# pytorch/ELF

Hardware: AMD Instinct MI355X
Metric: mcts_rollouts_per_sec (self-play, 19x19 Go, 8192 rollouts/move, bs 16) (higher is better)
Workload: dtype f32; 1 GPU; BASELINE configs[2]: MCTS self-play bs=16, 8192 rollouts/move, 20x256 fp16 net on PyTorch-ROCm, 2048 games/GPU in 1 group(s), window crosses a move boundary; games_per_gpu=2048, groups=1, board_size=19, mcts_threads=1, net_dtype=fp16, moves_in_window=2048, nodes_per_game=12288, node_bytes=6626, live_nodes=6241478, largest_tree=8184

## Files before the change

elf_amd/_lib.py:

```python
import ctypes as C
import os

HERE = os.path.dirname(os.path.abspath(__file__))
LIB_PATH = os.path.join(HERE, "lib", "libelf_amd.so")
ZOBRIST_BIN = os.path.join(HERE, "data", "zobrist21.bin")

_lib = None

KERNEL_SOURCES = ("go_board.cuh", "mcts.cuh", "train.cuh", "stl_emul.h", "engine_host.h", "elf_amd.hip", "mcts_capi.hip", "train_capi.hip",
                  "net_epilogue.hip", "Makefile")


def kernel_source_hash():
    import hashlib
    h = hashlib.sha256()
    for name in KERNEL_SOURCES:
        with open(os.path.join(HERE, "csrc", name), "rb") as f:
            h.update(name.encode() + b"\0" + f.read() + b"\0")
    return h.hexdigest()[:16]

_vp, _i, _i64, _f, _sz = C.c_void_p, C.c_int, C.c_int64, C.c_float, C.c_size_t
SIGNATURES = {
    "elfgo_create": (_i, [_i, _i, _i, _vp, C.POINTER(_vp)]),
    "elfgo_destroy": (_i, [_vp]),
    "elfgo_board_size": (_i, [_vp]),
    "elfgo_capacity": (_i, [_vp]),
    "elfgo_slot_bytes": (_sz, [_vp]),
    "elfgo_sync": (_i, [_vp, _vp]),
    "elfgo_reset": (_i, [_vp, _vp, _i, _vp]),
    "elfgo_copy": (_i, [_vp, _vp, _vp, _i, _vp]),
    "elfgo_forward": (_i, [_vp, _vp, _vp, _i, _vp, _vp]),
    "elfgo_legal_mask": (_i, [_vp, _vp, _i, _vp, _vp]),
    "elfgo_extract_agz": (_i, [_vp, _vp, _vp, _i, _vp, _i64, _vp]),
    "elfgo_extract_agz_fmt": (_i, [_vp, _vp, _vp, _i, _vp, _i64, _i, _vp]),
    "elfgo_evaluate": (_i, [_vp, _vp, _i, _f, _vp, _vp]),
    "elfgo_info": (_i, [_vp, _vp, _i, _vp, _vp]),
    "elfgo_export_board": (_i, [_vp, _vp, _i, _vp, _vp, _vp]),
    "elfgo_playout": (_i, [_vp, _vp, _vp, _i, _i, _vp, _vp]),
    "elfgo_setup": (_i, [_vp, _vp, _vp, _vp, _i, _vp, _vp]),
    "elfgo_area_map": (_i, [_vp, _vp, _i, _vp, _vp]),
    "elfgo_ladder_map": (_i, [_vp, _vp, _i, _vp, _vp, _vp]),
    "elfgo_own_create": (_i, [_vp, _i, C.POINTER(_vp)]),
    "elfgo_own_destroy": (_i, [_vp]),
    "elfgo_own_scratch_bytes": (_sz, [_vp]),
    "elfgo_own_run": (_i, [_vp, _vp, _vp, _i, _i, _i, _f, _vp, _vp, _vp]),
    "elfmcts_create": (_i, [_vp, _i, _i, _i, _vp, C.POINTER(_vp)]),
    "elfmcts_destroy": (_i, [_vp]),
    "elfmcts_set_options": (_i, [_vp, _vp]),
    "elfmcts_set_feature_format": (_i, [_vp, _i]),
    "elfmcts_get_feature_format": (_i, [_vp, C.POINTER(_i)]),
    "elfmcts_max_rollouts_per_step": (_i, []),
    "elfmcts_set_game_mask": (_i, [_vp, _vp]),
    "elfmcts_set_required_versions": (_i, [_vp, _vp]),
    "elfmcts_num_games": (_i, [_vp]),
    "elfmcts_edge_stride": (_i, [_vp]),
    "elfmcts_node_bytes": (_sz, [_vp]),
    "elfmcts_tree_bytes_per_game": (_sz, [_i, _i]),
    "elfmcts_tree_bytes_per_game2": (_sz, [_i, _i, _i, _i, _i]),
    "elfmcts_pool_info": (_i, [_vp, _vp, _i]),
    "elfmcts_count_live": (_i, [_vp, _vp]),
    "elfmcts_num_threads": (_i, [_vp]),
    "elfmcts_thread_draws": (_i, [_vp, _vp, _vp]),
    "elfmcts_clear": (_i, [_vp, _vp, _i, _vp]),
    "elfmcts_set_root": (_i, [_vp, _vp, _vp]),
    "elfmcts_set_d4": (_i, [_vp, _vp, _vp]),
    "elfmcts_dirichlet": (_i, [_vp, _vp, _vp, _f, _vp]),
    "elfmcts_select": (_i, [_vp, _vp, _vp, _i64, _vp, _vp]),
    "elfmcts_expand": (_i, [_vp, _vp, _i64, _vp, _vp, _i, _vp]),
    "elfmcts_root": (_i, [_vp, _vp, _vp, _vp, _vp, _vp, _vp, _vp]),
    "elfmcts_advance": (_i, [_vp, _vp, _vp]),
    "elfmcts_validate": (_i, [_vp, _vp]),
    "elfmcts_node_visits": (_i, [_vp, _vp]),
    "elfsp_create": (_i, [_vp, _i, _vp, C.POINTER(_vp)]),
    "elfsp_destroy": (_i, [_vp]),
    "elfsp_engine": (_vp, [_vp]),
    "elfsp_mcts": (_vp, [_vp]),
    "elfsp_ts_requests_deferred": (_i64, [_vp]),
    "elfsp_ts_games_deferred": (_i, [_vp]),
    "elfsp_max_rows": (_i, [_vp]),
    "elfsp_max_rows_actor": (_i, [_vp, _i]),
    "elfsp_mcts_actor": (_vp, [_vp, _i]),
    "elfsp_begin_step2": (_i, [_vp, _vp, _i64, _vp, _vp]),
    "elfsp_end_step2": (_i, [_vp, _vp, _i64, _vp, _vp, _vp]),
    "elfsp_last_rows2": (_i, [_vp, _vp]),
    "elfsp_set_request2": (_i, [_vp, _vp]),
    "elfsp_set_request3": (_i, [_vp, _vp, _vp]),
    "elfrec_sgf_parse": (_i, [_i, C.c_char_p, _vp, _vp, _i, _vp]),
    "elfrec_sgf_setup": (_i, [_i, C.c_char_p, _vp, _vp]),
    "elfrec_game_sgf": (_i64, [_vp, _vp, _i, _vp, _i, _f, C.c_char_p, C.c_char_p, C.c_char_p, C.c_char_p, _sz]),
    "elfrec_record_to_sgf": (_i64, [_vp, C.c_char_p, C.c_char_p, C.c_char_p, _sz, C.c_char_p, _sz]),
    "elfrec_client_create": (_i, [C.c_char_p, C.POINTER(_vp)]),
    "elfrec_client_destroy": (_i, [_vp]),
    "elfrec_client_feed": (_i, [_vp, C.c_char_p]),
    "elfrec_client_update_state": (_i, [_vp, _vp]),
    "elfrec_client_size": (_i, [_vp]),
    "elfrec_client_dump_and_clear": (_i64, [_vp, C.c_char_p, _sz]),
    "elfrec_parse_request_seq": (_i, [C.c_char_p, _vp, C.POINTER(_i64), _vp]),
    "elfrec_request_seq_to_json": (_i64, [_vp, _vp, _i64, C.c_char_p, _sz]),
    "elfsp_thread_states": (_i, [_vp, _vp, _i]),
    "elfrq_create": (_i, [_i, _i, _i, C.c_uint32, C.POINTER(_vp)]),
    "elfrq_destroy": (_i, [_vp]),
    "elfrq_insert": (_i, [_vp, C.c_int32, C.c_int32, _i, C.POINTER(C.c_int32)]),
    "elfrq_sizes": (_i, [_vp, _vp]),
    "elfrq_set_threads": (_i, [_vp, _i, _i64, C.c_uint64]),
    "elfrq_draw": (_i, [_vp, _i, _i, _vp, _vp, _vp]),
    "elfsp_progress": (_i, [_vp, _vp]),
    "elfsp_set_pick_seed": (_i, [_vp, C.c_uint32]),
    "elfsp_game_actor": (_i, [_vp, _i]),
    "elfsp_begin_step": (_i, [_vp, _vp, _i64, C.POINTER(_i), _vp]),
    "elfsp_end_step": (_i, [_vp, _vp, _i64, _vp, _vp, _vp]),
    "elfsp_last_rows": (_i, [_vp, C.POINTER(_i)]),
    "elfsp_set_request": (_i, [_vp, _i64, _i64, _f, _f, _i]),
    "elfsp_take_game_starts": (_i, [_vp, C.POINTER(_i64), C.POINTER(_i64)]),
    "elfsp_stats": (_i, [_vp, _vp]),
    "elfsp_games_finished": (_i64, [_vp]),
    "elfsp_search_log": (_i, [_vp, _i, _i, _vp, _vp, _vp, _vp, _vp]),
    "elfsp_play": (_i, [_vp, _vp, _vp]),
    "elfsp_preload": (_i, [_vp, _vp, _i, _i, _vp]),
    "elfsp_restart": (_i, [_vp, _vp, _i, _vp]),
    "elfsp_setup": (_i, [_vp, _vp, _i, _vp, _vp, _vp]),
    "elfsp_undo": (_i, [_vp, _vp, _i, _i, _vp]),
    "elfsp_finish": (_i, [_vp, _vp, _i, _i, _vp]),
    "elfsp_take_finished": (_i, [_vp, _vp, _i]),
    "elfsp_last_score": (_i, [_vp, _vp]),
    "elfsp_last_moves": (_i, [_vp, _vp]),
    "elfsp_records_pending": (_i, [_vp]),
    "elfsp_pop_record": (_i, [_vp, _vp, _sz, C.POINTER(_sz)]),
    "elftrain_create": (_i, [_vp, _i, _i, _i, C.c_uint32, C.POINTER(_vp)]),
    "elftrain_destroy": (_i, [_vp]),
    "elftrain_capacity": (_i, [_vp]),
    "elftrain_max_moves": (_i, [_vp]),
    "elftrain_num_records": (_i, [_vp]),
    "elftrain_put": (_i, [_vp, _i, _vp, _i, _f, _i64, _vp, _i, _vp, _i]),
    "elftrain_put_async": (_i, [_vp, _i, _vp, _i, _f, _i64, _vp, _i, _vp, _i, _vp]),
    "elftrain_set_keep_states": (_i, [_vp, _i]),
    "elftrain_draw": (_i, [_vp, _i, _i, _vp, _vp, _vp, _vp]),
    "elftrain_extract": (_i, [_vp, _vp, _vp, _vp, _i, _vp, _vp]),
    "elfrec_coords_to_sgfstr": (_i, [_i, _vp, _i, _vp, _sz]),
    "elfrec_sgfstr_to_coords": (_i, [_i, C.c_char_p, _vp, _i]),
    "elfrec_record_to_json": (_i, [_vp, _vp, _i, _vp, _i, _vp, _i, _f, _i, _i, C.c_uint64, C.c_uint64, _vp, _sz]),
    "elfrec_record_to_json2": (_i, [_vp, _vp, _vp, _i, _vp, _i, _vp, _i, _f, _i, _i, C.c_uint64, C.c_uint64, _vp, _sz]),
    "elfrec_quantise_policy": (_i, [_i, _vp, _vp, _i, _vp]),
    "elfnet_bias_act_f16": (_i, [_vp, _vp, _vp, _i64, _i, _i, _vp]),
    "elfnet_bias_act_bf16": (_i, [_vp, _vp, _vp, _i64, _i, _i, _vp]),
    "elfnet_conv3x3_f16": (_i, [_vp, _vp, _vp, _vp, _vp, _i64, _i, _i, _i, _i, _i, _i, _vp]),
    "elfgo_set_device": (_i, [_i]),
    "elfgo_get_device": (_i, [C.POINTER(_i)]),
    "elfgo_mem_info": (_i, [_i, C.POINTER(_sz), C.POINTER(_sz)]),
    "elfgo_pointer_kind": (_i, [_vp, C.POINTER(_i)]),
    "elfgo_memcpy2d_async": (_i, [_vp, _sz, _vp, _sz, _sz, _sz, _vp]),
    "elfgo_stream_sync": (_i, [_vp]),
    "elfgo_malloc": (_i, [C.POINTER(_vp), _sz]),
    "elfgo_free": (_i, [_vp]),
    "elfgo_memcpy_h2d": (_i, [_vp, _vp, _sz]),
    "elfgo_memcpy_d2h": (_i, [_vp, _vp, _sz]),
    "elfgo_error_string": (C.c_char_p, [_i]),
    "elfgo_version": (C.c_char_p, []),
}


def lib():
    global _lib
    if _lib is None:
        if not os.path.exists(LIB_PATH):
            raise ImportError(
                "elf_amd: %s not built. Run `python -c 'import __graft_entry__ as g; g.build()'` "
                "(or make -C elf_amd/csrc). There is no CPU fallback." % LIB_PATH
            )
        L = C.CDLL(LIB_PATH)
        for name, (res, args) in SIGNATURES.items():
            f = getattr(L, name)
            f.restype = res
            f.argtypes = args
        _lib = L
    return _lib


class ElfGoError(RuntimeError):
    pass


def check(status):
    if status != 0:
        raise ElfGoError("libelf_amd status %d: %s" % (status, lib().elfgo_error_string(status).decode()))
```

elf_amd/csrc/net_conv.hip:

```cpp
#include <hip/hip_runtime.h>
#include <stdint.h>

#include <array>

#if !__has_include("ck/ck.hpp")
#error "net_conv.hip needs Composable Kernel's headers (ck/ck.hpp, shipped with ROCm under <rocm>/include/ck): there is no build of libelf_amd.so without the fused trunk convolution"
#endif
#include "ck/ck.hpp"
#include "ck/tensor_operation/gpu/device/convolution_forward_specialization.hpp"
#include "ck/tensor_operation/gpu/device/gemm_specialization.hpp"
#include "ck/tensor_operation/gpu/device/impl/device_grouped_conv_fwd_multiple_abd_xdl_cshuffle.hpp"
#include "ck/tensor_operation/gpu/device/tensor_layout.hpp"
#include "ck/tensor_operation/gpu/element/element_wise_operation.hpp"

#include "../../include/elf_amd.h"

namespace {

using F16 = ck::half_t;
using F32 = float;
template <ck::index_t... Is>
using S = ck::Sequence<Is...>;
using PassThrough = ck::tensor_operation::element_wise::PassThrough;
namespace lay = ck::tensor_layout::convolution;

struct BiasResAct {
  int relu;
  template <typename E, typename C, typename D0>
  __host__ __device__ void operator()(E& e, const C& c, const D0& bias) const {
    float v = ck::type_convert<float>(ck::type_convert<F16>(c));
    v += ck::type_convert<float>(bias);
    if (relu) v = fmaxf(v, 0.0f);
    e = ck::type_convert<E>(v);
  }
  template <typename E, typename C, typename D0, typename D1>
  __host__ __device__ void operator()(E& e, const C& c, const D0& bias, const D1& res) const {
    float v = ck::type_convert<float>(ck::type_convert<F16>(c));
    v += ck::type_convert<float>(bias);
    v += ck::type_convert<float>(res);
    if (relu) v = fmaxf(v, 0.0f);
    e = ck::type_convert<E>(v);
  }
};

constexpr auto kConvDefault = ck::tensor_operation::device::ConvolutionForwardSpecialization::Default;
constexpr auto kMNKPadding = ck::tensor_operation::device::GemmSpecialization::MNKPadding;

template <typename DsLayout, typename DsTypes>
using ConvA = ck::tensor_operation::device::DeviceGroupedConvFwdMultipleABD_Xdl_CShuffle<
    2, lay::NHWGC, lay::GKYXC, DsLayout, lay::NHWGK, F16, F16, F32, F16, DsTypes, F16, PassThrough, PassThrough, BiasResAct,
    kConvDefault, kMNKPadding, 1, 256, 256, 128, 32, 8, 8, 32, 32, 4, 2,
    S<4, 64, 1>, S<1, 0, 2>, S<1, 0, 2>, 2, 8, 8, 1,
    S<4, 64, 1>, S<1, 0, 2>, S<1, 0, 2>, 2, 8, 8, 1,
    1, 1, S<1, 32, 1, 8>, 8>;

using DsBias = ck::Tuple<lay::G_K>;
using DsBiasRes = ck::Tuple<lay::G_K, lay::NHWGK>;
using T1 = ck::Tuple<F16>;
using T2 = ck::Tuple<F16, F16>;

struct DevGuard {
  int prev = -1;
  explicit DevGuard(int dev) {
    int cur = -1;
    if (hipGetDevice(&cur) == hipSuccess && cur != dev && hipSetDevice(dev) == hipSuccess) prev = cur;
  }
  ~DevGuard() { if (prev >= 0) (void)hipSetDevice(prev); }
  DevGuard(const DevGuard&) = delete;
  DevGuard& operator=(const DevGuard&) = delete;
};

struct Shape { int n, h, w, c, k; };

template <typename Op, int ND>
int run(const void* x, const void* w, const std::array<const void*, ND>& ds, void* y, const Shape& s, int relu, hipStream_t stream,
        bool launch) {
  using A5 = std::array<ck::index_t, 5>;
  using A2 = std::array<ck::index_t, 2>;
  const int n = s.n, h = s.h, wd = s.w, c = s.c, k = s.k;
  const A5 xl{1, n, c, h, wd}, xs{c, h * wd * c, 1, wd * c, c};
  const A5 wl{1, k, c, 3, 3}, ws{k * 9 * c, 9 * c, 1, 3 * c, c};
  const A5 yl{1, n, k, h, wd}, ys{k, h * wd * k, 1, wd * k, k};
  const A5 bs{k, 0, 1, 0, 0};
  std::array<A5, ND> dl, dst;
  dl[0] = yl; dst[0] = bs;
  if (ND == 2) { dl[ND - 1] = yl; dst[ND - 1] = ys; }
  const A2 one{1, 1};
  try {
    auto arg = Op::MakeArgument(x, w, ds, y, xl, xs, wl, ws, dl, dst, yl, ys, one, one, one, one, PassThrough{}, PassThrough{},
                                BiasResAct{relu});
    if (!Op::IsSupportedArgument(arg)) return ELFGO_E_BADARG;
    if (!launch) return 0;
    auto inv = Op::MakeInvoker();
    (void)inv.Run(arg, StreamConfig{stream, false});
  } catch (...) {
    hipError_t e = hipGetLastError();
    return e == hipSuccess ? (int)hipErrorLaunchFailure : (int)e;
  }
  hipError_t e = hipGetLastError();
  return e == hipSuccess ? 0 : (int)e;
}

}

extern "C" __attribute__((visibility("hidden"))) int elfnet_conv3x3_native_f16(const void* x, const void* w, const void* bias,
                                                                               const void* res, void* y, int64_t rows, int h, int wd,
                                                                               int c, int k, int relu, hipStream_t stream);

extern "C" int elfnet_conv3x3_f16(const void* x, const void* w, const void* bias, const void* res, void* y, int64_t rows, int h, int wd,
                                  int c, int k, int relu, int algo, void* stream) {
  if (!x || !w || !bias || !y || rows < 0 || h <= 0 || wd <= 0 || c <= 0 || k <= 0) return ELFGO_E_BADARG;
  if ((c & 7) != 0 || (k & 7) != 0 || (algo != 0 && algo != 1)) return ELFGO_E_BADARG;
  if ((((uintptr_t)x | (uintptr_t)w | (uintptr_t)bias | (uintptr_t)res | (uintptr_t)y) & 15) != 0) return ELFGO_E_BADARG;
  if (y == x || y == res) return ELFGO_E_BADARG;
  const int64_t cmax = c > k ? c : k;
  if (rows * h * wd * cmax >= ((int64_t)1 << 30) || (int64_t)k * 9 * c >= ((int64_t)1 << 30)) return ELFGO_E_BADARG;
  if (rows == 0) return 0;
  hipPointerAttribute_t at;
  if (hipPointerGetAttributes(&at, x) != hipSuccess) { (void)hipGetLastError(); return ELFGO_E_BADARG; }
  DevGuard _dg(at.device);
  const Shape s{(int)rows, h, wd, c, k};
  hipStream_t st = (hipStream_t)stream;
  if (algo == 1) return elfnet_conv3x3_native_f16(x, w, bias, res, y, rows, h, wd, c, k, relu, st);
  if (res) return run<ConvA<DsBiasRes, T2>, 2>(x, w, {bias, res}, y, s, relu, st, true);
  return run<ConvA<DsBias, T1>, 1>(x, w, {bias}, y, s, relu, st, true);
}
```

elf_amd/csrc/net_conv3x3.hip:

```cpp
#include <hip/hip_runtime.h>
#include <stdint.h>

#include "../../include/elf_amd.h"


namespace {

typedef _Float16 half8 __attribute__((ext_vector_type(8)));
typedef _Float16 half4 __attribute__((ext_vector_type(4)));
typedef float floatx16 __attribute__((ext_vector_type(16)));

constexpr int kTileM = 256;
constexpr int kTileN = 256;
constexpr int kThreads = 512;
constexpr int kOperandBytes = 256 * 128;
constexpr int kBufBytes = 2 * kOperandBytes;
constexpr int kLdsBytes = 2 * kBufBytes;

__device__ __attribute__((aligned(128))) unsigned char g_zero_line[128] = {0};

typedef const __attribute__((address_space(1))) void* gptr_t;
typedef __attribute__((address_space(3))) void* lptr_t;

__device__ __forceinline__ void stage16(const char* src, char* lds_base) {
  __builtin_amdgcn_global_load_lds((gptr_t)src, (lptr_t)lds_base, 16, 0, 0);
}

template <int kN, bool kLgkm>
__device__ __forceinline__ void wait_staged() {
  if constexpr (kLgkm) asm volatile("s_waitcnt vmcnt(%0) lgkmcnt(0)" ::"n"(kN) : "memory");
  else asm volatile("s_waitcnt vmcnt(%0)" ::"n"(kN) : "memory");
}
__device__ __forceinline__ void raw_barrier() {
  __builtin_amdgcn_s_barrier();
  asm volatile("" ::: "memory");
  __builtin_amdgcn_sched_barrier(0);
}
template <int kV> struct Mode { static constexpr int v = kV; };

template <bool kHasRes>
__global__ __launch_bounds__(kThreads, 2) void k_conv3x3_f16(const char* __restrict__ x, const char* __restrict__ w,
                                                             const _Float16* __restrict__ bias, const _Float16* __restrict__ res,
                                                             _Float16* __restrict__ y, int M, int H, int W, int Cin, int K, int relu) {
  __shared__ __attribute__((aligned(128))) char lds[kLdsBytes];
  const int tid = threadIdx.x, lane = tid & 63, wv = __builtin_amdgcn_readfirstlane(tid >> 6);
  const int kbase = blockIdx.y * kTileN;
  const int tile = blockIdx.x;

  uint32_t xoff[4], woff[4], xmask[4];
  const unsigned char* zsrc = g_zero_line + (lane & 7) * 16;
#pragma unroll
  for (int j = 0; j < 4; ++j) {
    const int hf = j >> 1, i = j & 1;
    const int r = i * 128 + hf * 64 + wv * 8 + (lane >> 3);
    const int p = tile * kTileM + r;
    uint32_t m = 0;
    if (p < M) {
      const int rem = p % (H * W), hh = rem / W, ww = rem - hh * W;
#pragma unroll
      for (int tap = 0; tap < 9; ++tap) {
        const int dy = tap / 3 - 1, dx = tap % 3 - 1;
        if ((unsigned)(hh + dy) < (unsigned)H && (unsigned)(ww + dx) < (unsigned)W) m |= 1u << tap;
      }
    }
    xmask[j] = m;
    xoff[j] = (uint32_t)p * (uint32_t)(Cin * 2) + (((lane & 7) ^ ((r >> 1) & 7)) << 4);
    const int rw = (i * 2 + (wv >> 2)) * 64 + hf * 32 + (wv & 3) * 8 + (lane >> 3);
    woff[j] = (uint32_t)(kbase + rw) * (uint32_t)(9 * Cin * 2) + (((lane & 7) ^ ((rw >> 1) & 7)) << 4);
  }
  auto stage_x = [&](int hf, int tap, int kc, int buf) {
    const int dy = tap / 3 - 1, dx = tap - (tap / 3) * 3 - 1;
    const uint32_t d = (uint32_t)((dy * W + dx) * Cin * 2 + kc * 128);
#pragma unroll
    for (int i = 0; i < 2; ++i)
      stage16(((xmask[hf * 2 + i] >> tap) & 1) ? x + (uint32_t)(xoff[hf * 2 + i] + d) : (const char*)zsrc,
              lds + buf * kBufBytes + (i * 128 + hf * 64 + wv * 8) * 128);
  };
  auto stage_w = [&](int hf, int tap, int kc, int buf) {
    const uint32_t d = (uint32_t)(tap * Cin * 2 + kc * 128);
#pragma unroll
    for (int i = 0; i < 2; ++i)
      stage16(w + (uint32_t)(woff[hf * 2 + i] + d),
              lds + buf * kBufBytes + kOperandBytes + ((i * 2 + (wv >> 2)) * 64 + hf * 32 + (wv & 3) * 8) * 128);
  };

  const int wm = wv >> 2, wn = wv & 3;
  const int fr = lane & 31, fh = lane >> 5;
  const int sw = (fr >> 1) & 7;
  const int xrow = (wm * 128 + fr) * 128;
  const int wrow = kOperandBytes + (wn * 64 + fr) * 128;
  int cs[4];
#pragma unroll
  for (int kk = 0; kk < 4; ++kk) cs[kk] = (((kk >> 1) * 4 + fh * 2 + (kk & 1)) ^ sw) << 4;
  auto ldx = [&](const char* b, int mt, int kk) { return *(const half8*)(b + xrow + mt * 4096 + cs[kk]); };
  auto ldw = [&](const char* b, int nt, int kk) { return *(const half8*)(b + wrow + nt * 4096 + cs[kk]); };

  floatx16 acc[4][2];
#pragma unroll
  for (int mt = 0; mt < 4; ++mt)
#pragma unroll
    for (int nt = 0; nt < 2; ++nt)
#pragma unroll
      for (int e = 0; e < 16; ++e) acc[mt][nt][e] = 0.0f;

  const int kchunks = Cin >> 6, ktiles = 9 * kchunks;
  half8 xf[2][4], wa[4], wb[4];
  int tap1 = 0, kc1 = 1, tap2 = 0, kc2 = 2;
  if (kchunks == 1) { tap1 = 1; kc1 = 0; tap2 = 2; kc2 = 0; }
  else if (kchunks == 2) { tap2 = 1; kc2 = 0; }
  stage_x(0, 0, 0, 0); stage_w(0, 0, 0, 0); stage_w(1, 0, 0, 0); stage_x(1, 0, 0, 0);
  stage_x(0, tap1, kc1, 1); stage_w(0, tap1, kc1, 1); stage_w(1, tap1, kc1, 1);
  wait_staged<8, false>();
  raw_barrier();

  auto ktile = [&](auto mode, int t) {
    constexpr int kMode = decltype(mode)::v;
    const int cur = t & 1, nxt = cur ^ 1;
    const char* b = lds + cur * kBufBytes;
#pragma unroll
    for (int kk = 0; kk < 4; ++kk) {
      wa[kk] = ldw(b, 0, kk);
      xf[0][kk] = ldx(b, 0, kk);
      xf[1][kk] = ldx(b, 1, kk);
      wb[kk] = ldw(b, 1, kk);
    }
    if constexpr (kMode <= 1) stage_x(1, tap1, kc1, nxt);
    wait_staged<kMode == 2 ? 0 : 8, true>();
    raw_barrier();
    __builtin_amdgcn_s_setprio(1);
#pragma unroll
    for (int kk = 0; kk < 4; ++kk) {
      acc[0][0] = __builtin_amdgcn_mfma_f32_32x32x16_f16(wa[kk], xf[0][kk], acc[0][0], 0, 0, 0);
      acc[1][0] = __builtin_amdgcn_mfma_f32_32x32x16_f16(wa[kk], xf[1][kk], acc[1][0], 0, 0, 0);
      acc[0][1] = __builtin_amdgcn_mfma_f32_32x32x16_f16(wb[kk], xf[0][kk], acc[0][1], 0, 0, 0);
      acc[1][1] = __builtin_amdgcn_mfma_f32_32x32x16_f16(wb[kk], xf[1][kk], acc[1][1], 0, 0, 0);
    }
    __builtin_amdgcn_s_setprio(0);
    __builtin_amdgcn_sched_barrier(0);
    raw_barrier();
#pragma unroll
    for (int kk = 0; kk < 4; ++kk) {
      xf[0][kk] = ldx(b, 2, kk);
      xf[1][kk] = ldx(b, 3, kk);
    }
    if constexpr (kMode == 0) { stage_x(0, tap2, kc2, cur); stage_w(0, tap2, kc2, cur); stage_w(1, tap2, kc2, cur); }
    wait_staged<kMode == 0 ? 8 : kMode == 1 ? 2 : 0, true>();
    raw_barrier();
    __builtin_amdgcn_s_setprio(1);
#pragma unroll
    for (int kk = 0; kk < 4; ++kk) {
      acc[2][0] = __builtin_amdgcn_mfma_f32_32x32x16_f16(wa[kk], xf[0][kk], acc[2][0], 0, 0, 0);
      acc[3][0] = __builtin_amdgcn_mfma_f32_32x32x16_f16(wa[kk], xf[1][kk], acc[3][0], 0, 0, 0);
      acc[2][1] = __builtin_amdgcn_mfma_f32_32x32x16_f16(wb[kk], xf[0][kk], acc[2][1], 0, 0, 0);
      acc[3][1] = __builtin_amdgcn_mfma_f32_32x32x16_f16(wb[kk], xf[1][kk], acc[3][1], 0, 0, 0);
    }
    __builtin_amdgcn_s_setprio(0);
    __builtin_amdgcn_sched_barrier(0);
    raw_barrier();
  };
  const int late = __builtin_amdgcn_readfirstlane(tid >> 8);
  if (late) raw_barrier();
  for (int t = 0; t < ktiles - 2; ++t) {
    ktile(Mode<0>{}, t);
    tap1 = tap2; kc1 = kc2;
    if (++kc2 == kchunks) { kc2 = 0; ++tap2; }
  }
  ktile(Mode<1>{}, ktiles - 2);
  ktile(Mode<2>{}, ktiles - 1);
  if (!late) raw_barrier();

  __syncthreads();
#pragma unroll
  for (int mt = 0; mt < 4; ++mt)
#pragma unroll
    for (int nt = 0; nt < 2; ++nt) {
      const int pos = wm * 128 + mt * 32 + fr;
#pragma unroll
      for (int g = 0; g < 4; ++g) {
        const int ch = wn * 64 + nt * 32 + g * 8 + fh * 4;
        half4 hv;
#pragma unroll
        for (int e = 0; e < 4; ++e) hv[e] = (_Float16)acc[mt][nt][g * 4 + e];
        *(half4*)(lds + pos * 512 + (((ch >> 3) ^ (pos & 31)) << 4) + ((ch >> 2) & 1) * 8) = hv;
      }
    }
  const int q = tid & 31;
  const half8 bv = *(const half8*)(bias + kbase + q * 8);
  if constexpr (kHasRes) {
    half8 rv[16];
#pragma unroll
    for (int it = 0; it < 16; ++it) {
      const int p = tile * kTileM + it * 16 + (tid >> 5);
      rv[it] = *(const half8*)(res + (size_t)(p < M ? p : M - 1) * K + kbase + q * 8);
    }
    __syncthreads();
#pragma unroll
    for (int it = 0; it < 16; ++it) {
      const int pos = it * 16 + (tid >> 5);
      const int p = tile * kTileM + pos;
      const half8 cv = *(const half8*)(lds + pos * 512 + ((q ^ (pos & 31)) << 4));
      half8 ov;
#pragma unroll
      for (int e = 0; e < 8; ++e) {
        float v = (float)cv[e];
        v += (float)bv[e];
        v += (float)rv[it][e];
        if (relu) v = fmaxf(v, 0.0f);
        ov[e] = (_Float16)v;
      }
      if (p < M) *(half8*)(y + (size_t)p * K + kbase + q * 8) = ov;
    }
  } else {
    __syncthreads();
#pragma unroll 4
    for (int it = 0; it < 16; ++it) {
      const int pos = it * 16 + (tid >> 5);
      const int p = tile * kTileM + pos;
      if (p < M) {
        const half8 cv = *(const half8*)(lds + pos * 512 + ((q ^ (pos & 31)) << 4));
        half8 ov;
#pragma unroll
        for (int e = 0; e < 8; ++e) {
          float v = (float)cv[e];
          v += (float)bv[e];
          if (relu) v = fmaxf(v, 0.0f);
          ov[e] = (_Float16)v;
        }
        *(half8*)(y + (size_t)p * K + kbase + q * 8) = ov;
      }
    }
  }
}

}

extern "C" __attribute__((visibility("hidden"))) int elfnet_conv3x3_native_f16(const void* x, const void* w, const void* bias,
                                                                               const void* res, void* y, int64_t rows, int h, int wd,
                                                                               int c, int k, int relu, hipStream_t stream) {
  if ((c & 63) != 0 || (k & 255) != 0) return ELFGO_E_BADARG;
  const int64_t m = rows * h * wd;
  const dim3 grid((unsigned)((m + kTileM - 1) / kTileM), (unsigned)(k / kTileN));
  if (res)
    hipLaunchKernelGGL(k_conv3x3_f16<true>, grid, dim3(kThreads), 0, stream, (const char*)x, (const char*)w, (const _Float16*)bias,
                       (const _Float16*)res, (_Float16*)y, (int)m, h, wd, c, k, relu);
  else
    hipLaunchKernelGGL(k_conv3x3_f16<false>, grid, dim3(kThreads), 0, stream, (const char*)x, (const char*)w, (const _Float16*)bias,
                       (const _Float16*)nullptr, (_Float16*)y, (int)m, h, wd, c, k, relu);
  hipError_t e = hipGetLastError();
  return e == hipSuccess ? 0 : (int)e;
}
```

include/elf_amd.h:

```cpp
#ifndef ELF_AMD_H_
#define ELF_AMD_H_
#include <stddef.h>
#include <stdint.h>

#ifdef __cplusplus
extern "C" {
#endif

typedef struct ElfGoEngine ElfGoEngine;

#define ELFGO_E_BADARG (-1)
#define ELFGO_E_BADSIZE (-2)
#define ELFGO_E_NOMEM (-3)
#define ELFGO_E_NODATA (-4)

#define ELFGO_INFO_WORDS 16

int elfgo_create(int board_size, int capacity, int device, const uint64_t* zobrist_host, ElfGoEngine** out);
int elfgo_destroy(ElfGoEngine* e);
int elfgo_board_size(const ElfGoEngine* e);
int elfgo_capacity(const ElfGoEngine* e);
size_t elfgo_slot_bytes(const ElfGoEngine* e);
int elfgo_sync(ElfGoEngine* e, void* stream);

// ... 115 lines not shown
  int32_t following_pass;
  int32_t reserved1;
} ElfSpOptions;
#define ELFSP_PICK_MOST_VISITED 0
#define ELFSP_PICK_STRONGEST_PRIOR 1
#define ELFSP_PICK_UNIFORM_RANDOM 2
#define ELFSP_ACTOR_BLACK 0
#define ELFSP_ACTOR_WHITE 1

typedef struct ElfSpSearch {
  int32_t game, move_played, best_action, total_visits, n_edges;
  float root_value, max_score, predicted_value;
} ElfSpSearch;

int elfsp_create(const ElfSpOptions* opt, int device, const uint64_t* zobrist_host, ElfSelfPlay** out);
int elfsp_destroy(ElfSelfPlay* sp);
ElfGoEngine* elfsp_engine(ElfSelfPlay* sp);
ElfMcts* elfsp_mcts(ElfSelfPlay* sp);
int64_t elfsp_ts_requests_deferred(const ElfSelfPlay* sp);
int elfsp_ts_games_deferred(const ElfSelfPlay* sp);
int elfsp_max_rows(const ElfSelfPlay* sp);
int elfsp_max_rows_actor(const ElfSelfPlay* sp, int actor);
ElfMcts* elfsp_mcts_actor(ElfSelfPlay* sp, int actor);
int elfsp_begin_step(ElfSelfPlay* sp, void* s_dst, int64_t stride_elems, int* n_rows, void* stream);
int elfsp_end_step(ElfSelfPlay* sp, const float* pi, int64_t pi_stride_floats, const float* value, const int64_t* rv, void* stream);
int elfsp_last_rows(ElfSelfPlay* sp, int* n_rows);
int elfsp_begin_step2(ElfSelfPlay* sp, void* const* s_dst, int64_t stride_elems, int* n_rows, void* stream);
int elfsp_end_step2(ElfSelfPlay* sp, const float* const* pi, int64_t pi_stride_floats, const float* const* value,
                    const int64_t* const* rv, void* stream);
int elfsp_last_rows2(ElfSelfPlay* sp, int* n_rows);
typedef struct ElfTsOptions {
  int32_t max_num_moves, num_threads, num_rollouts_per_thread, num_rollouts_per_batch;
  int32_t verbose, verbose_time, persistent_tree, pick_method ;
  int64_t seed;
  float root_epsilon, root_alpha;
  int32_t virtual_loss;
  int32_t use_prior, unexplored_q_zero, root_unexplored_q_zero;
  float c_puct;
  char log_prefix[60];
} ElfTsOptions;
typedef struct ElfSpRequest {
  int64_t black_ver, white_ver;
  float black_resign_thres, white_resign_thres, never_resign_prob;
  int32_t num_game_thread_used;
  int32_t player_swap;
  int32_t async;
  int32_t client_type;
} ElfSpRequest;
int elfsp_set_request2(ElfSelfPlay* sp, const ElfSpRequest* request);
int elfsp_set_request3(ElfSelfPlay* sp, const ElfSpRequest* request, const ElfTsOptions* mcts_opt);
int elfsp_set_request(ElfSelfPlay* sp, int64_t black_ver, int64_t white_ver, float resign_thres, float never_resign_prob, int async);
int elfsp_set_pick_seed(ElfSelfPlay* sp, uint32_t seed);
int elfsp_progress(const ElfSelfPlay* sp, int64_t* out6);
int elfsp_game_actor(const ElfSelfPlay* sp, int game);
int elfsp_take_game_starts(ElfSelfPlay* sp, int64_t* black_ver, int64_t* white_ver);
int elfsp_stats(ElfSelfPlay* sp, int64_t* out);
int elfsp_play(ElfSelfPlay* sp, const int32_t* moves_host, void* stream);
int elfsp_preload(ElfSelfPlay* sp, const uint16_t* moves_host, int n, int move_to, void* stream);
int elfsp_setup(ElfSelfPlay* sp, const int32_t* games_host, int n, const uint8_t* stones_host,
                const uint8_t* next_player_host, void* stream);
int elfsp_undo(ElfSelfPlay* sp, const int32_t* games_host, int n, int count, void* stream);
#define ELFSP_FR_RESIGN 0
#define ELFSP_FR_TWO_PASSES 1
#define ELFSP_FR_MAX_STEP 2
#define ELFSP_FR_CLEAR 3
#define ELFSP_FR_ILLEGAL 4
int elfsp_finish(ElfSelfPlay* sp, const int32_t* games_host, int n, int reason, void* stream);
int elfsp_restart(ElfSelfPlay* sp, const int32_t* games_host, int n, void* stream);
int elfsp_take_finished(ElfSelfPlay* sp, float* out_host, int cap);
int elfsp_last_score(const ElfSelfPlay* sp, float* out_host);
int elfsp_last_moves(const ElfSelfPlay* sp, int32_t* out_host);
int elfsp_records_pending(const ElfSelfPlay* sp);
int elfsp_pop_record(ElfSelfPlay* sp, char* buf, size_t cap, size_t* len);
int64_t elfsp_games_finished(const ElfSelfPlay* sp);
int elfsp_search_log(const ElfSelfPlay* sp, int first, int n, ElfSpSearch* rec, int32_t* coord, int32_t* visits, float* prior,
                     float* reward);

typedef struct ElfReplay ElfReplay;

typedef struct ElfTrainBatch {
  void* s;
  int64_t s_stride;
  int32_t s_format;
  int32_t num_future_actions;
  int64_t* offline_a;
  float* winner;
  float* mcts_scores;
  float* predicted_value;
  int32_t* move_idx;
  int32_t* num_move;
  int32_t* aug_code;
  int64_t* selfplay_ver;
} ElfTrainBatch;

int elftrain_create(ElfGoEngine* e, int capacity, int max_moves, int with_policies, uint32_t seed, ElfReplay** out);
int elftrain_destroy(ElfReplay* r);
int elftrain_capacity(const ElfReplay* r);
int elftrain_max_moves(const ElfReplay* r);
int elftrain_num_records(const ElfReplay* r);
int elftrain_put(ElfReplay* r, int slot, const uint16_t* moves_host, int num_moves, float reward, int64_t black_ver,
                 const uint8_t* policies_host, int num_policies, const float* values_host, int num_values);
int elftrain_put_async(ElfReplay* r, int slot, const uint16_t* moves_host, int num_moves, float reward, int64_t black_ver,
                       const uint8_t* policies_host, int num_policies, const float* values_host, int num_values, void* stream);
int elftrain_set_keep_states(ElfReplay* r, int on);
int elftrain_draw(ElfReplay* r, int n, int num_future_actions, int32_t* rec, int32_t* move_to, int32_t* d4, void* stream);
typedef struct ElfSgfHeader {
  int32_t size, handi, winner ;
  float komi, win_margin;
} ElfSgfHeader;
int elfrec_sgf_parse(int board_size, const char* text, int32_t* players, uint16_t* coords, int cap, ElfSgfHeader* header);
int elfrec_sgf_setup(int board_size, const char* text, uint8_t* stones, ElfSgfHeader* header);
int64_t elfrec_game_sgf(const ElfSpOptions* opt, const uint16_t* moves, int num_moves, const float* values, int num_values,
                        float final_value, const char* filename, const char* git_hash, const char* git_staged, char* out, size_t cap);
int64_t elfrec_record_to_sgf(const ElfSpOptions* opt, const char* record_json, const char* prefix, char* name_out, size_t name_cap,
                             char* out, size_t cap);
typedef struct ElfThreadState {
  int32_t thread_id, seq, move_idx, reserved;
  int64_t black, white;
} ElfThreadState;
typedef struct ElfClientRecords ElfClientRecords;
int elfrec_client_create(const char* identity, ElfClientRecords** out);
int elfrec_client_destroy(ElfClientRecords* c);
int elfrec_client_feed(ElfClientRecords* c, const char* record_json);
int elfrec_client_update_state(ElfClientRecords* c, const ElfThreadState* state);
int elfrec_client_size(const ElfClientRecords* c);
int64_t elfrec_client_dump_and_clear(ElfClientRecords* c, char* out, size_t cap);
int elfrec_parse_request_seq(const char* json_text, ElfSpRequest* request, int64_t* seq, ElfTsOptions* mcts_opt);
int64_t elfrec_request_seq_to_json(const ElfSpRequest* request, const ElfTsOptions* mcts_opt, int64_t seq, char* out, size_t cap);
int elfsp_thread_states(const ElfSelfPlay* sp, ElfThreadState* out, int capacity);
typedef struct ElfReaderQueues ElfReaderQueues;
int elfrq_create(int num_reader, int queue_min_size, int queue_max_size, uint32_t insert_seed, ElfReaderQueues** out);
int elfrq_destroy(ElfReaderQueues* q);
int elfrq_insert(ElfReaderQueues* q, int32_t slot, int32_t num_moves, int black_win, int32_t* evicted);
int elfrq_sizes(const ElfReaderQueues* q, int32_t* per_queue);
int elfrq_set_threads(ElfReaderQueues* q, int num_threads, int64_t seed, uint64_t job_hash);
int elfrq_draw(ElfReaderQueues* q, int num_acts, int num_future_actions, int32_t* slot, int32_t* move_to, int32_t* d4);
int elftrain_extract(ElfReplay* r, const int32_t* rec, const int32_t* move_to, const int32_t* d4, int n, const ElfTrainBatch* out,
                     void* stream);

int elfrec_coords_to_sgfstr(int board_size, const uint16_t* coords, int n, char* out, size_t cap);
int elfrec_sgfstr_to_coords(int board_size, const char* sgf, uint16_t* out, int cap);
int elfrec_record_to_json(const ElfSpOptions* opt, const uint16_t* moves, int num_moves, const uint8_t* policies, int num_policies,
                          const float* values, int num_values, float reward, int never_resign, int seq, uint64_t thread_id,
                          uint64_t timestamp, char* out, size_t cap);
int elfrec_record_to_json2(const ElfSpOptions* opt, const ElfSpRequest* request, const uint16_t* moves, int num_moves,
                           const uint8_t* policies, int num_policies, const float* values, int num_values, float reward, int never_resign,
                           int seq, uint64_t thread_id, uint64_t timestamp, char* out, size_t cap);
int elfrec_quantise_policy(int board_size, const int32_t* coord, const float* prob, int n, uint8_t* out);

int elfnet_bias_act_f16(void* x, const void* bias, const void* res, int64_t rows, int channels, int relu, void* stream);
int elfnet_bias_act_bf16(void* x, const void* bias, const void* res, int64_t rows, int channels, int relu, void* stream);
int elfnet_conv3x3_f16(const void* x, const void* w, const void* bias, const void* res, void* y,
                       int64_t rows, int h, int wd, int c, int k, int relu, int algo, void* stream);

int elfgo_set_device(int device);
int elfgo_get_device(int* device);
int elfgo_mem_info(int device, size_t* free_bytes, size_t* total_bytes);
int elfgo_pointer_kind(const void* p, int* device);
int elfgo_memcpy2d_async(void* dst, size_t dst_pitch, const void* src, size_t src_pitch, size_t width_bytes, size_t rows, void* stream);
int elfgo_stream_sync(void* stream);
int elfgo_malloc(void** dptr, size_t bytes);
int elfgo_free(void* dptr);
int elfgo_memcpy_h2d(void* dst, const void* src_host, size_t bytes);
int elfgo_memcpy_d2h(void* dst_host, const void* src, size_t bytes);
const char* elfgo_error_string(int status);
const char* elfgo_version(void);

#ifdef __cplusplus
}
#endif
#endif
```

Measured before the change: 63030 rollouts/s.

## Make native conv3x3 kernel persistent with half-width tail units and per-wave epilogue

Converts the native fp16 3x3 conv kernel from one workgroup per output tile to a persistent grid sized to the CU count. Each workgroup loops over (tile, channel-block) units and prefetches the next unit's operands across unit boundaries. Leftover units are split into half-width channel halves so the final wave stays balanced. The epilogue is rewritten to go through per-wave LDS shuffle space, which adds LDS use and may reduce occupancy, and the added control flow in the inner loop could cost scheduling quality. This only runs when algo==1 is selected, which the default self-play path may not use.

```diff
diff --git a/elf_amd/_lib.py b/elf_amd/_lib.py
--- a/elf_amd/_lib.py
+++ b/elf_amd/_lib.py
@@ -144,6 +144,7 @@
     "elfnet_bias_act_f16": (_i, [_vp, _vp, _vp, _i64, _i, _i, _vp]),
     "elfnet_bias_act_bf16": (_i, [_vp, _vp, _vp, _i64, _i, _i, _vp]),
     "elfnet_conv3x3_f16": (_i, [_vp, _vp, _vp, _vp, _vp, _i64, _i, _i, _i, _i, _i, _i, _vp]),
+    "elfnet_conv3x3_f16_wgs": (_i, [_vp, _vp, _vp, _vp, _vp, _i64, _i, _i, _i, _i, _i, _i, _i, _vp]),
     "elfgo_set_device": (_i, [_i]),
     "elfgo_get_device": (_i, [C.POINTER(_i)]),
     "elfgo_mem_info": (_i, [_i, C.POINTER(_sz), C.POINTER(_sz)]),
diff --git a/elf_amd/csrc/net_conv.hip b/elf_amd/csrc/net_conv.hip
--- a/elf_amd/csrc/net_conv.hip
+++ b/elf_amd/csrc/net_conv.hip
@@ -105,10 +105,12 @@
 
 extern "C" __attribute__((visibility("hidden"))) int elfnet_conv3x3_native_f16(const void* x, const void* w, const void* bias,
                                                                                const void* res, void* y, int64_t rows, int h, int wd,
-                                                                               int c, int k, int relu, hipStream_t stream);
+                                                                               int c, int k, int relu, int workgroups, int device,
+                                                                               hipStream_t stream);
 
-extern "C" int elfnet_conv3x3_f16(const void* x, const void* w, const void* bias, const void* res, void* y, int64_t rows, int h, int wd,
-                                  int c, int k, int relu, int algo, void* stream) {
+extern "C" int elfnet_conv3x3_f16_wgs(const void* x, const void* w, const void* bias, const void* res, void* y, int64_t rows, int h,
+                                      int wd, int c, int k, int relu, int algo, int workgroups, void* stream) {
+  if (workgroups < 0) return ELFGO_E_BADARG;
   if (!x || !w || !bias || !y || rows < 0 || h <= 0 || wd <= 0 || c <= 0 || k <= 0) return ELFGO_E_BADARG;
   if ((c & 7) != 0 || (k & 7) != 0 || (algo != 0 && algo != 1)) return ELFGO_E_BADARG;
   if ((((uintptr_t)x | (uintptr_t)w | (uintptr_t)bias | (uintptr_t)res | (uintptr_t)y) & 15) != 0) return ELFGO_E_BADARG;
@@ -121,7 +123,12 @@
   DevGuard _dg(at.device);
   const Shape s{(int)rows, h, wd, c, k};
   hipStream_t st = (hipStream_t)stream;
-  if (algo == 1) return elfnet_conv3x3_native_f16(x, w, bias, res, y, rows, h, wd, c, k, relu, st);
+  if (algo == 1) return elfnet_conv3x3_native_f16(x, w, bias, res, y, rows, h, wd, c, k, relu, workgroups, at.device, st);
   if (res) return run<ConvA<DsBiasRes, T2>, 2>(x, w, {bias, res}, y, s, relu, st, true);
   return run<ConvA<DsBias, T1>, 1>(x, w, {bias}, y, s, relu, st, true);
 }
+
+extern "C" int elfnet_conv3x3_f16(const void* x, const void* w, const void* bias, const void* res, void* y, int64_t rows, int h, int wd,
+                                  int c, int k, int relu, int algo, void* stream) {
+  return elfnet_conv3x3_f16_wgs(x, w, bias, res, y, rows, h, wd, c, k, relu, algo, 0, stream);
+}
diff --git a/elf_amd/csrc/net_conv3x3.hip b/elf_amd/csrc/net_conv3x3.hip
--- a/elf_amd/csrc/net_conv3x3.hip
+++ b/elf_amd/csrc/net_conv3x3.hip
@@ -1,5 +1,7 @@
 #include <hip/hip_runtime.h>
 #include <stdint.h>
+
+#include <atomic>
 
 #include "../../include/elf_amd.h"
 
@@ -15,7 +17,8 @@
 constexpr int kThreads = 512;
 constexpr int kOperandBytes = 256 * 128;
 constexpr int kBufBytes = 2 * kOperandBytes;
-constexpr int kLdsBytes = 2 * kBufBytes;
+constexpr int kShuffleBytes = 8 * 4096;
+constexpr int kLdsBytes = 2 * kBufBytes + kShuffleBytes;
 
 __device__ __attribute__((aligned(128))) unsigned char g_zero_line[128] = {0};
 
@@ -36,21 +39,43 @@
   asm volatile("" ::: "memory");
   __builtin_amdgcn_sched_barrier(0);
 }
-template <int kV> struct Mode { static constexpr int v = kV; };
+template <int kV> struct Int { static constexpr int v = kV; };
+struct Seg { int nt2, s1, s2, w1, w2; };
+__device__ __forceinline__ Seg seg_of(int half, int left, int next) {
+  if (half) return left >= 2 ? Seg{0, 1, 1, 6, 6} : left == 1 ? Seg{0, 1, 0, 6, 2} : Seg{0, 0, 0, 0, 0};
+  if (left >= 2 || next == 1) return Seg{1, 1, 2, 8, 8};
+  if (next == 2) return left == 1 ? Seg{1, 1, 1, 8, 6} : Seg{1, 1, 1, 6, 6};
+  return left == 1 ? Seg{1, 1, 0, 8, 2} : Seg{1, 0, 0, 0, 0};
+}
+__device__ __forceinline__ void wait_staged_n(int n) {
+  if (n == 8) wait_staged<8, true>();
+  else if (n == 6) wait_staged<6, true>();
+  else if (n == 2) wait_staged<2, true>();
+  else wait_staged<0, true>();
+}
 
 template <bool kHasRes>
 __global__ __launch_bounds__(kThreads, 2) void k_conv3x3_f16(const char* __restrict__ x, const char* __restrict__ w,
                                                              const _Float16* __restrict__ bias, const _Float16* __restrict__ res,
-                                                             _Float16* __restrict__ y, int M, int H, int W, int Cin, int K, int relu) {
+                                                             _Float16* __restrict__ y, int M, int H, int W, int Cin, int K, int relu,
+                                                             int nfull, int nhalf2) {
   __shared__ __attribute__((aligned(128))) char lds[kLdsBytes];
   const int tid = threadIdx.x, lane = tid & 63, wv = __builtin_amdgcn_readfirstlane(tid >> 6);
-  const int kbase = blockIdx.y * kTileN;
-  const int tile = blockIdx.x;
+  const int wg = blockIdx.x, grid = gridDim.x, kblocks = K >> 8;
+  const int myfull = wg < nfull ? (nfull - 1 - wg) / grid + 1 : 0;
+  const int myhalf = wg < nhalf2 ? 1 : 0;
+  auto unit_of = [&](int i, int* tile, int* ch, int* half) {
+    const int u = i < myfull ? wg + i * grid : nfull + (wg >> 1);
+    *tile = u / kblocks;
+    *half = i < myfull ? 0 : 1;
+    *ch = (u - *tile * kblocks) * kTileN + (i < myfull ? 0 : (wg & 1) * (kTileN / 2));
+  };
 
   uint32_t xoff[4], woff[4], xmask[4];
   const unsigned char* zsrc = g_zero_line + (lane & 7) * 16;
-#pragma unroll
-  for (int j = 0; j < 4; ++j) {
+  auto lane_here = [&]() { int l = lane; asm volatile("" : "+v"(l)); return l; };
+  auto set_x = [&](int j, int tile) {
+    const int lane = lane_here();
     const int hf = j >> 1, i = j & 1;
     const int r = i * 128 + hf * 64 + wv * 8 + (lane >> 3);
     const int p = tile * kTileM + r;
@@ -65,9 +90,17 @@
     }
     xmask[j] = m;
     xoff[j] = (uint32_t)p * (uint32_t)(Cin * 2) + (((lane & 7) ^ ((r >> 1) & 7)) << 4);
-    const int rw = (i * 2 + (wv >> 2)) * 64 + hf * 32 + (wv & 3) * 8 + (lane >> 3);
-    woff[j] = (uint32_t)(kbase + rw) * (uint32_t)(9 * Cin * 2) + (((lane & 7) ^ ((rw >> 1) & 7)) << 4);
-  }
+  };
+  auto set_w = [&](int ch, int half) {
+    const int lane = lane_here();
+#pragma unroll
+    for (int j = 0; j < 4; ++j) {
+      const int hf = j >> 1, i = j & 1;
+      const int rw = (i * 2 + (wv >> 2)) * 64 + hf * 32 + (wv & 3) * 8 + (lane >> 3);
+      const int row = half ? ch + (rw >> 6) * 32 + (rw & 31) : ch + rw;
+      woff[j] = (uint32_t)row * (uint32_t)(9 * Cin * 2) + (((lane & 7) ^ ((rw >> 1) & 7)) << 4);
+    }
+  };
   auto stage_x = [&](int hf, int tap, int kc, int buf) {
     const int dy = tap / 3 - 1, dx = tap - (tap / 3) * 3 - 1;
     const uint32_t d = (uint32_t)((dy * W + dx) * Cin * 2 + kc * 128);
@@ -96,156 +129,218 @@
   auto ldw = [&](const char* b, int nt, int kk) { return *(const half8*)(b + wrow + nt * 4096 + cs[kk]); };
 
   floatx16 acc[4][2];
-#pragma unroll
-  for (int mt = 0; mt < 4; ++mt)
-#pragma unroll
-    for (int nt = 0; nt < 2; ++nt)
-#pragma unroll
-      for (int e = 0; e < 16; ++e) acc[mt][nt][e] = 0.0f;
+  auto zero_acc = [&]() {
+#pragma unroll
+    for (int mt = 0; mt < 4; ++mt)
+#pragma unroll
+      for (int nt = 0; nt < 2; ++nt)
+#pragma unroll
+        for (int e = 0; e < 16; ++e) acc[mt][nt][e] = 0.0f;
+  };
+
+  int tile, ch, half;
+  unit_of(0, &tile, &ch, &half);
+#pragma unroll
+  for (int j = 0; j < 4; ++j) set_x(j, tile);
+  set_w(ch, half);
+  half8 bv;
+  auto load_bias = [&](int c0, int nt) {
+    bv = *(const half8*)(bias + c0 + wn * (32 * nt) + (lane & (4 * nt - 1)) * 8);
+    asm volatile("s_waitcnt vmcnt(0)" : "+v"(bv)::"memory");
+  };
+  load_bias(ch, half ? 1 : 2);
 
   const int kchunks = Cin >> 6, ktiles = 9 * kchunks;
   half8 xf[2][4], wa[4], wb[4];
   int tap1 = 0, kc1 = 1, tap2 = 0, kc2 = 2;
   if (kchunks == 1) { tap1 = 1; kc1 = 0; tap2 = 2; kc2 = 0; }
   else if (kchunks == 2) { tap2 = 1; kc2 = 0; }
-  stage_x(0, 0, 0, 0); stage_w(0, 0, 0, 0); stage_w(1, 0, 0, 0); stage_x(1, 0, 0, 0);
-  stage_x(0, tap1, kc1, 1); stage_w(0, tap1, kc1, 1); stage_w(1, tap1, kc1, 1);
-  wait_staged<8, false>();
+  stage_x(0, 0, 0, 0); stage_w(0, 0, 0, 0);
+  if (!half) stage_w(1, 0, 0, 0);
+  stage_x(1, 0, 0, 0);
+  stage_x(0, tap1, kc1, 1); stage_w(0, tap1, kc1, 1);
+  if (!half) {
+    stage_w(1, tap1, kc1, 1);
+    wait_staged<8, false>();
+  } else {
+    wait_staged<6, false>();
+  }
   raw_barrier();
 
-  auto ktile = [&](auto mode, int t) {
-    constexpr int kMode = decltype(mode)::v;
-    const int cur = t & 1, nxt = cur ^ 1;
+  int par = 0;
+  int ntile = 0, nch = 0, nhalf = 0;
+  auto ktile = [&](const Seg sg, int prep) {
+    const int cur = par, nxt = cur ^ 1;
     const char* b = lds + cur * kBufBytes;
 #pragma unroll
     for (int kk = 0; kk < 4; ++kk) {
       wa[kk] = ldw(b, 0, kk);
       xf[0][kk] = ldx(b, 0, kk);
       xf[1][kk] = ldx(b, 1, kk);
-      wb[kk] = ldw(b, 1, kk);
-    }
-    if constexpr (kMode <= 1) stage_x(1, tap1, kc1, nxt);
-    wait_staged<kMode == 2 ? 0 : 8, true>();
+    }
+    if (sg.nt2) {
+#pragma unroll
+      for (int kk = 0; kk < 4; ++kk) wb[kk] = ldw(b, 1, kk);
+    }
+    if (sg.s1) stage_x(1, tap1, kc1, nxt);
+    wait_staged_n(sg.w1);
     raw_barrier();
     __builtin_amdgcn_s_setprio(1);
 #pragma unroll
     for (int kk = 0; kk < 4; ++kk) {
       acc[0][0] = __builtin_amdgcn_mfma_f32_32x32x16_f16(wa[kk], xf[0][kk], acc[0][0], 0, 0, 0);
       acc[1][0] = __builtin_amdgcn_mfma_f32_32x32x16_f16(wa[kk], xf[1][kk], acc[1][0], 0, 0, 0);
-      acc[0][1] = __builtin_amdgcn_mfma_f32_32x32x16_f16(wb[kk], xf[0][kk], acc[0][1], 0, 0, 0);
-      acc[1][1] = __builtin_amdgcn_mfma_f32_32x32x16_f16(wb[kk], xf[1][kk], acc[1][1], 0, 0, 0);
+      if (sg.nt2) {
+        acc[0][1] = __builtin_amdgcn_mfma_f32_32x32x16_f16(wb[kk], xf[0][kk], acc[0][1], 0, 0, 0);
+        acc[1][1] = __builtin_amdgcn_mfma_f32_32x32x16_f16(wb[kk], xf[1][kk], acc[1][1], 0, 0, 0);
+      }
     }
     __builtin_amdgcn_s_setprio(0);
     __builtin_amdgcn_sched_barrier(0);
+    if (prep == 2) { set_x(2, ntile); set_x(3, ntile); }
     raw_barrier();
 #pragma unroll
     for (int kk = 0; kk < 4; ++kk) {
       xf[0][kk] = ldx(b, 2, kk);
       xf[1][kk] = ldx(b, 3, kk);
     }
-    if constexpr (kMode == 0) { stage_x(0, tap2, kc2, cur); stage_w(0, tap2, kc2, cur); stage_w(1, tap2, kc2, cur); }
-    wait_staged<kMode == 0 ? 8 : kMode == 1 ? 2 : 0, true>();
+    if (sg.s2 >= 1) { stage_x(0, tap2, kc2, cur); stage_w(0, tap2, kc2, cur); }
+    if (sg.s2 == 2) stage_w(1, tap2, kc2, cur);
+    wait_staged_n(sg.w2);
     raw_barrier();
     __builtin_amdgcn_s_setprio(1);
 #pragma unroll
     for (int kk = 0; kk < 4; ++kk) {
       acc[2][0] = __builtin_amdgcn_mfma_f32_32x32x16_f16(wa[kk], xf[0][kk], acc[2][0], 0, 0, 0);
       acc[3][0] = __builtin_amdgcn_mfma_f32_32x32x16_f16(wa[kk], xf[1][kk], acc[3][0], 0, 0, 0);
-      acc[2][1] = __builtin_amdgcn_mfma_f32_32x32x16_f16(wb[kk], xf[0][kk], acc[2][1], 0, 0, 0);
-      acc[3][1] = __builtin_amdgcn_mfma_f32_32x32x16_f16(wb[kk], xf[1][kk], acc[3][1], 0, 0, 0);
+      if (sg.nt2) {
+        acc[2][1] = __builtin_amdgcn_mfma_f32_32x32x16_f16(wb[kk], xf[0][kk], acc[2][1], 0, 0, 0);
+        acc[3][1] = __builtin_amdgcn_mfma_f32_32x32x16_f16(wb[kk], xf[1][kk], acc[3][1], 0, 0, 0);
+      }
     }
     __builtin_amdgcn_s_setprio(0);
     __builtin_amdgcn_sched_barrier(0);
+    if (prep == 1) { set_x(0, ntile); set_x(1, ntile); set_w(nch, nhalf); }
     raw_barrier();
-  };
-  const int late = __builtin_amdgcn_readfirstlane(tid >> 8);
-  if (late) raw_barrier();
-  for (int t = 0; t < ktiles - 2; ++t) {
-    ktile(Mode<0>{}, t);
+    par ^= 1;
     tap1 = tap2; kc1 = kc2;
-    if (++kc2 == kchunks) { kc2 = 0; ++tap2; }
-  }
-  ktile(Mode<1>{}, ktiles - 2);
-  ktile(Mode<2>{}, ktiles - 1);
-  if (!late) raw_barrier();
-
-  __syncthreads();
-#pragma unroll
-  for (int mt = 0; mt < 4; ++mt)
-#pragma unroll
-    for (int nt = 0; nt < 2; ++nt) {
-      const int pos = wm * 128 + mt * 32 + fr;
-#pragma unroll
-      for (int g = 0; g < 4; ++g) {
-        const int ch = wn * 64 + nt * 32 + g * 8 + fh * 4;
-        half4 hv;
-#pragma unroll
-        for (int e = 0; e < 4; ++e) hv[e] = (_Float16)acc[mt][nt][g * 4 + e];
-        *(half4*)(lds + pos * 512 + (((ch >> 3) ^ (pos & 31)) << 4) + ((ch >> 2) & 1) * 8) = hv;
-      }
-    }
-  const int q = tid & 31;
-  const half8 bv = *(const half8*)(bias + kbase + q * 8);
-  if constexpr (kHasRes) {
-    half8 rv[16];
-#pragma unroll
-    for (int it = 0; it < 16; ++it) {
-      const int p = tile * kTileM + it * 16 + (tid >> 5);
-      rv[it] = *(const half8*)(res + (size_t)(p < M ? p : M - 1) * K + kbase + q * 8);
-    }
-    __syncthreads();
-#pragma unroll
-    for (int it = 0; it < 16; ++it) {
-      const int pos = it * 16 + (tid >> 5);
-      const int p = tile * kTileM + pos;
-      const half8 cv = *(const half8*)(lds + pos * 512 + ((q ^ (pos & 31)) << 4));
-      half8 ov;
-#pragma unroll
-      for (int e = 0; e < 8; ++e) {
-        float v = (float)cv[e];
-        v += (float)bv[e];
-        v += (float)rv[it][e];
-        if (relu) v = fmaxf(v, 0.0f);
-        ov[e] = (_Float16)v;
-      }
-      if (p < M) *(half8*)(y + (size_t)p * K + kbase + q * 8) = ov;
-    }
-  } else {
-    __syncthreads();
-#pragma unroll 4
-    for (int it = 0; it < 16; ++it) {
-      const int pos = it * 16 + (tid >> 5);
-      const int p = tile * kTileM + pos;
-      if (p < M) {
-        const half8 cv = *(const half8*)(lds + pos * 512 + ((q ^ (pos & 31)) << 4));
+    if (++kc2 == kchunks) { kc2 = 0; if (++tap2 == 9) tap2 = 0; }
+  };
+
+  auto epilogue = [&](auto ntc, int tile, int c0) {
+    constexpr int kNt = decltype(ntc)::v, kCpr = 4 * kNt, kRpi = 64 / kCpr, kIts = 32 / kRpi;
+    const int lane = lane_here(), fr = lane & 31, fh = lane >> 5, sw = (fr >> 1) & 7;
+    const int q = lane & (kCpr - 1), rl = lane / kCpr;
+    char* cw = lds + 2 * kBufBytes + wv * 4096;
+    const int pbase = tile * kTileM + wm * 128, cbase = c0 + wn * (32 * kNt) + q * 8;
+    half8 rv[4][kIts];
+    if constexpr (kHasRes) {
+#pragma unroll
+      for (int mt = 0; mt < 4; ++mt)
+#pragma unroll
+        for (int it = 0; it < kIts; ++it) {
+          const int p = pbase + mt * 32 + it * kRpi + rl;
+          rv[mt][it] = *(const half8*)(res + (size_t)(p < M ? p : M - 1) * K + cbase);
+        }
+    }
+#pragma unroll
+    for (int mt = 0; mt < 4; ++mt) {
+#pragma unroll
+      for (int nt = 0; nt < kNt; ++nt)
+#pragma unroll
+        for (int g = 0; g < 4; ++g) {
+          half4 hv;
+#pragma unroll
+          for (int e = 0; e < 4; ++e) hv[e] = (_Float16)acc[mt][nt][g * 4 + e];
+          *(half4*)(cw + fr * 128 + (((nt * 4 + g) ^ sw) << 4) + fh * 8) = hv;
+        }
+      if constexpr (kHasRes) {
+        if (mt == 0) {
+#pragma unroll
+          for (int m2 = 0; m2 < 4; ++m2)
+#pragma unroll
+            for (int it = 0; it < kIts; ++it) asm volatile("" : "+v"(rv[m2][it]));
+        }
+      }
+      asm volatile("s_waitcnt lgkmcnt(0)" ::: "memory");
+#pragma unroll
+      for (int it = 0; it < kIts; ++it) {
+        const int row = it * kRpi + rl;
+        const int p = pbase + mt * 32 + row;
+        const half8 cv = *(const half8*)(cw + row * 128 + ((q ^ ((row >> 1) & 7)) << 4));
         half8 ov;
 #pragma unroll
         for (int e = 0; e < 8; ++e) {
           float v = (float)cv[e];
           v += (float)bv[e];
+          if constexpr (kHasRes) v += (float)rv[mt][it][e];
           if (relu) v = fmaxf(v, 0.0f);
           ov[e] = (_Float16)v;
         }
-        *(half8*)(y + (size_t)p * K + kbase + q * 8) = ov;
-      }
-    }
+        if (p < M) *(half8*)(y + (size_t)p * K + cbase) = ov;
+      }
+      asm volatile("s_waitcnt lgkmcnt(0)" ::: "memory");
+    }
+  };
+
+  const int late = __builtin_amdgcn_readfirstlane(tid >> 8);
+  if (late) raw_barrier();
+  for (int i = 0; i < myfull + myhalf; ++i) {
+    const int next = i + 1 < myfull ? 1 : i + 1 < myfull + myhalf ? 2 : 0;
+    if (next) unit_of(i + 1, &ntile, &nch, &nhalf);
+    zero_acc();
+    for (int t = 0; t < ktiles; ++t) {
+      const int left = ktiles - 1 - t;
+      ktile(seg_of(half, left, next), next == 0 ? 0 : left == 2 ? 1 : left == 1 ? 2 : 0);
+    }
+    if (half) epilogue(Int<1>{}, tile, ch);
+    else epilogue(Int<2>{}, tile, ch);
+    if (next && (nch != ch || nhalf)) load_bias(nch, nhalf ? 1 : 2);
+    tile = ntile; ch = nch; half = nhalf;
   }
+  if (!late) raw_barrier();
+}
+
+struct UnitPlan { int grid, nfull, nhalf2; };
+UnitPlan plan_units(int64_t units, int64_t workgroups) {
+  const int64_t r = units % workgroups;
+  const bool split = r > 0 && 2 * r <= workgroups;
+  UnitPlan p;
+  p.nfull = (int)(split ? units - r : units);
+  p.nhalf2 = (int)(split ? 2 * r : 0);
+  p.grid = (int)(units >= workgroups ? workgroups : split ? 2 * r : units);
+  return p;
+}
+
+int cu_count(int device) {
+  static std::atomic<int> cached[64];
+  if (device < 0 || device >= 64) return 0;
+  int n = cached[device].load(std::memory_order_relaxed);
+  if (n == 0) {
+    if (hipDeviceGetAttribute(&n, hipDeviceAttributeMultiprocessorCount, device) != hipSuccess || n <= 0) { (void)hipGetLastError(); return 0; }
+    cached[device].store(n, std::memory_order_relaxed);
+  }
+  return n;
 }
 
 }
 
 extern "C" __attribute__((visibility("hidden"))) int elfnet_conv3x3_native_f16(const void* x, const void* w, const void* bias,
                                                                                const void* res, void* y, int64_t rows, int h, int wd,
-                                                                               int c, int k, int relu, hipStream_t stream) {
-  if ((c & 63) != 0 || (k & 255) != 0) return ELFGO_E_BADARG;
+                                                                               int c, int k, int relu, int workgroups, int device,
+                                                                               hipStream_t stream) {
+  if ((c & 63) != 0 || (k & 255) != 0 || workgroups < 0) return ELFGO_E_BADARG;
+  if (workgroups == 0) workgroups = cu_count(device);
+  if (workgroups <= 0) return ELFGO_E_BADARG;
   const int64_t m = rows * h * wd;
-  const dim3 grid((unsigned)((m + kTileM - 1) / kTileM), (unsigned)(k / kTileN));
+  const UnitPlan pl = plan_units((m + kTileM - 1) / kTileM * (k / kTileN), workgroups);
+  const dim3 grid((unsigned)pl.grid);
   if (res)
     hipLaunchKernelGGL(k_conv3x3_f16<true>, grid, dim3(kThreads), 0, stream, (const char*)x, (const char*)w, (const _Float16*)bias,
-                       (const _Float16*)res, (_Float16*)y, (int)m, h, wd, c, k, relu);
+                       (const _Float16*)res, (_Float16*)y, (int)m, h, wd, c, k, relu, pl.nfull, pl.nhalf2);
   else
     hipLaunchKernelGGL(k_conv3x3_f16<false>, grid, dim3(kThreads), 0, stream, (const char*)x, (const char*)w, (const _Float16*)bias,
-                       (const _Float16*)nullptr, (_Float16*)y, (int)m, h, wd, c, k, relu);
+                       (const _Float16*)nullptr, (_Float16*)y, (int)m, h, wd, c, k, relu, pl.nfull, pl.nhalf2);
   hipError_t e = hipGetLastError();
   return e == hipSuccess ? 0 : (int)e;
 }
diff --git a/include/elf_amd.h b/include/elf_amd.h
--- a/include/elf_amd.h
+++ b/include/elf_amd.h
@@ -291,6 +291,8 @@
 int elfnet_bias_act_bf16(void* x, const void* bias, const void* res, int64_t rows, int channels, int relu, void* stream);
 int elfnet_conv3x3_f16(const void* x, const void* w, const void* bias, const void* res, void* y,
                        int64_t rows, int h, int wd, int c, int k, int relu, int algo, void* stream);
+int elfnet_conv3x3_f16_wgs(const void* x, const void* w, const void* bias, const void* res, void* y,
+                           int64_t rows, int h, int wd, int c, int k, int relu, int algo, int workgroups, void* stream);
 
 int elfgo_set_device(int device);
 int elfgo_get_device(int* device);
```

New measurement: 57020 rollouts/s. 9.5% lower.
